# jfkirk/tensorrec

Hardware: NVIDIA H100
Metric: predict_rank_pairs_per_s (higher is better)
Workload: dtype f32 (1 fp16 wgmma filter pass with a certified bound + re-scoring of the survivors from the 22-bit split operands, fp32 accumulate)

## Files before the change

tensorrec_b200/csrc/filter_tc.cuh:

```cuda
#pragma once

#include "common.cuh"

namespace trk {

constexpr uint32_t kWarpStageBytes = 32 * 32 * 4u;
constexpr uint32_t kAccStageBytes = 4 * kWarpStageBytes;
constexpr float kMarginFactor = 1.5f * 0.0009765625f;
constexpr float kBiasUlps = 4.0f * 1.1920929e-7f;
constexpr float kThetaMargins = 2.25f;
constexpr int kGiveUpOverflows = 8;

struct AdmitCtx {
  const float* bias;
  const int32_t* perm;
  int32_t id_offset;
  int32_t n_items;
  int32_t k;
};

template <class Row>
__device__ __forceinline__ void set_tau(Row& r) {
  const float t = (r.theta - r.ubias) * r.inv_c;
  r.tau = t - 8.0f * 1.1920929e-7f * fabsf(t) - 1e-30f;
}

__device__ __forceinline__ float ldg_nc_f32(const float* p) {
  float v;
  asm volatile("ld.global.nc.f32 %0, [%1];" : "=f"(v) : "l"(p));
  return v;
}
__device__ __forceinline__ int32_t ldg_nc_s32(const int32_t* p) {
  int32_t v;
  asm volatile("ld.global.nc.s32 %0, [%1];" : "=r"(v) : "l"(p));
  return v;
}

__device__ __forceinline__ float acc_max_16(const uint32_t* acc, float (&g)[4]) {
#pragma unroll
  for (int q = 0; q < 4; ++q)
    g[q] = fmaxf(fmaxf(__uint_as_float(acc[4 * q]), __uint_as_float(acc[4 * q + 1])),
                 fmaxf(__uint_as_float(acc[4 * q + 2]), __uint_as_float(acc[4 * q + 3])));
  return fmaxf(fmaxf(g[0], g[1]), fmaxf(g[2], g[3]));
}
__device__ __forceinline__ float acc_max_16(const uint32_t* acc) {
  float g[4];
  return acc_max_16(acc, g);
}

__device__ __forceinline__ uint32_t pass_mask_16(const uint32_t* acc, const float (&g)[4], float bmax_scaled,
                                                 float tau) {
  uint32_t mask = 0;
#pragma unroll
  for (int q = 0; q < 4; ++q) {
    if (g[q] + bmax_scaled > tau) {
      const uint32_t b0 = (__uint_as_float(acc[4 * q + 0]) + bmax_scaled > tau) ? (1u << (4 * q + 0)) : 0u;
      const uint32_t b1 = (__uint_as_float(acc[4 * q + 1]) + bmax_scaled > tau) ? (1u << (4 * q + 1)) : 0u;
      const uint32_t b2 = (__uint_as_float(acc[4 * q + 2]) + bmax_scaled > tau) ? (1u << (4 * q + 2)) : 0u;
      const uint32_t b3 = (__uint_as_float(acc[4 * q + 3]) + bmax_scaled > tau) ? (1u << (4 * q + 3)) : 0u;
      mask |= (b0 | b1) | (b2 | b3);
    }
  }
  return mask;
}

__device__ __forceinline__ int filter_owned_row(int warp_in_group, int lane) {
  return 16 * warp_in_group + (lane & 15) + 64 * (lane >> 4);
}

template <int c>
__device__ __forceinline__ float chunk_row_max(const float (&acc0)[32], const float (&acc1)[32], int lane) {
  float m[4];
#pragma unroll
  for (int s = 0; s < 2; ++s) {
    const int i = 16 * c + 2 * s;
    m[s] = fmaxf(fmaxf(fmaxf(acc0[i], acc0[i + 1]), fmaxf(acc0[i + 4], acc0[i + 5])),
                 fmaxf(fmaxf(acc0[i + 8], acc0[i + 9]), fmaxf(acc0[i + 12], acc0[i + 13])));
    m[2 + s] = fmaxf(fmaxf(fmaxf(acc1[i], acc1[i + 1]), fmaxf(acc1[i + 4], acc1[i + 5])),
                     fmaxf(fmaxf(acc1[i + 8], acc1[i + 9]), fmaxf(acc1[i + 12], acc1[i + 13])));
  }
  const bool b0 = (lane & 1) != 0, b1 = (lane & 2) != 0;
  const float k0 = fmaxf(b0 ? m[1] : m[0], __shfl_xor_sync(0xffffffffu, b0 ? m[0] : m[1], 1));
  const float k1 = fmaxf(b0 ? m[3] : m[2], __shfl_xor_sync(0xffffffffu, b0 ? m[2] : m[3], 1));
  const float r = fmaxf(b1 ? k1 : k0, __shfl_xor_sync(0xffffffffu, b1 ? k0 : k1, 2));
  return __shfl_sync(0xffffffffu, r, 4 * (lane & 7) + (lane >> 3));
}

__device__ __forceinline__ uint32_t stage_swizzle(int g) { return 4u * static_cast<uint32_t>(((g & 3) << 1) | (g >> 2)); }
__device__ __forceinline__ void f_sts32(uint32_t addr, float v) {
  asm volatile("st.shared.f32 [%0], %1;" ::"r"(addr), "f"(v) : "memory");
}

template <int c>
__device__ __forceinline__ void stage_warp_chunk(const float (&acc0)[32], const float (&acc1)[32], uint32_t stage,
                                                 int lane) {
  __syncwarp();
  const int g = lane >> 2;
  const uint32_t col0 = 2u * static_cast<uint32_t>(lane & 3) ^ stage_swizzle(g);
  const uint32_t row_g = stage + 128u * g;
#pragma unroll
  for (int j = 0; j < 4; ++j) {
    const uint32_t a = row_g + 4u * (col0 ^ (8u * j));
#pragma unroll
    for (int s = 0; s < 2; ++s) {
      const int i = 16 * c + 4 * j + 2 * s;
      asm volatile("st.shared.v2.f32 [%0], {%1, %2};" ::"r"(a + 1024u * s), "f"(acc0[i]), "f"(acc0[i + 1]) : "memory");
      asm volatile("st.shared.v2.f32 [%0], {%1, %2};" ::"r"(a + 1024u * (2 + s)), "f"(acc1[i]), "f"(acc1[i + 1])
                   : "memory");
    }
  }
  __syncwarp();
}
__device__ __forceinline__ void load_staged_row(uint32_t stage, int lane, uint32_t (&v)[32]) {
  const uint32_t row = stage + 128u * lane, sw = stage_swizzle(lane & 7);
#pragma unroll
  for (uint32_t q = 0; q < 8; ++q)
    asm volatile("ld.shared.v4.b32 {%0, %1, %2, %3}, [%4];"
                 : "=r"(v[4 * q]), "=r"(v[4 * q + 1]), "=r"(v[4 * q + 2]), "=r"(v[4 * q + 3])
                 : "r"(row + 4u * ((4u * q) ^ sw))
                 : "memory");
}

inline __device__ __noinline__ int32_t excl_mask_chunk(const int32_t* indptr, const int32_t* pos, int64_t u,
                                                       int32_t base, uint32_t stage, int lane) {
  const uint32_t row = stage + 128u * lane, sw = stage_swizzle(lane & 7);
  const int hi = __ldg(indptr + u + 1);
  int i = excl_lower_bound(pos, __ldg(indptr + u), hi, base);
  int32_t e = i < hi ? __ldg(pos + i) : 0x7fffffff;
  while (e < base + 32) {
    f_sts32(row + 4u * (static_cast<uint32_t>(e - base) ^ sw), -__int_as_float(0x7f800000));
    ++i;
    e = i < hi ? __ldg(pos + i) : 0x7fffffff;
  }
  return e;
}

template <int kNKB>
__device__ __forceinline__ void filter_mma_half(float (&acc0)[32], float (&acc1)[32], uint32_t a_base, uint32_t b_slot,
                                                int h) {
  wgmma_fence();
#pragma unroll
  for (int kb = 0; kb < kNKB; ++kb) {
#pragma unroll
    for (int ks = 0; ks < kKBlock / kMmaK; ++ks) {
      const uint64_t db = wgmma_desc_k_major_sw128(b_slot + kb * kBTileBytes + h * (kBTileBytes / 2)) + 2u * ks;
      const uint64_t da = wgmma_desc_k_major_sw128(a_base + kb * kATileBytes) + 2u * ks;
      const uint32_t accumulate = static_cast<uint32_t>(kb > 0 || ks > 0);
      wgmma_m64n64k16_f16(acc0, da, db, accumulate);
      wgmma_m64n64k16_f16(acc1, da + ((kATileBytes / 2) >> 4), db, accumulate);
    }
  }
  wgmma_commit();
  wgmma_wait<0>();
}

__device__ __forceinline__ uint32_t wide_key(float s) {
  const uint32_t u = __float_as_uint(s);
  return (u & 0x80000000u) ? ~u : (u | 0x80000000u);
}
__device__ __forceinline__ float wide_unkey(uint32_t key) {
  return __uint_as_float((key & 0x80000000u) ? (key & 0x7fffffffu) : ~key);
}

}
```

tensorrec_b200/csrc/score_filter_tc.cu:

```cuda
#include <stdlib.h>

#include "filter_tc.cuh"

namespace trk {

constexpr int kBufEntries = 32;
constexpr int kKeepMax = 16;
constexpr int kFilterMaxK = 12;

struct FilterParams {
  const __half* user_split;
  const float* user_scale;
  const float* user_bias;
  const float* user_norm;
  const float* item_bias;
  const float* block_bias_max;
  const float* block_bias_min;
  const int32_t* item_perm;
  const float* item_stats;
  int64_t n_users;
  int64_t n_items;
  int32_t n_kblocks;
  int32_t d_pad;
  int32_t n_stages;
  int32_t k;
  int32_t n_splits;
  int32_t tiles_per_split;
  int32_t n_tiles;
  int32_t n_user_pairs;
  int32_t item_id_offset;
  int32_t tile_end_trigger;
  float* cand_score;
  int32_t* cand_item;
  float* row_theta;
  const int32_t* excl_indptr;
  const int32_t* excl_pos;
};

struct FilterLayout {
  uint32_t a_off, b_off, buf_off, acc_off, bar_off, total;
};
__host__ __device__ inline FilterLayout filter_layout(int n_kblocks, int n_stages) {
  FilterLayout L;
  L.a_off = 0;
  L.b_off = L.a_off + 2u * static_cast<uint32_t>(n_kblocks) * kATileBytes;
  L.buf_off = L.b_off + static_cast<uint32_t>(n_stages) * kBTileBytes;
  L.acc_off = L.buf_off + 2u * kBlockM * kBufEntries * 8u;
  L.bar_off = L.acc_off + 2u * kAccStageBytes;
  L.total = L.bar_off + 512u;
  return L;
}

__device__ __forceinline__ void f_sts64(uint32_t addr, float s, int32_t id) {
  asm volatile("st.shared.v2.b32 [%0], {%1, %2};" ::"r"(addr), "r"(__float_as_uint(s)), "r"(id) : "memory");
}
__device__ __forceinline__ void f_lds64(uint32_t addr, float* s, int32_t* id) {
  uint32_t a, b;
  asm volatile("ld.shared.v2.b32 {%0, %1}, [%2];" : "=r"(a), "=r"(b) : "r"(addr) : "memory");
  *s = __uint_as_float(a);
  *id = static_cast<int32_t>(b);
}
__device__ __forceinline__ bool cand_before(float xs, int32_t xi, float ys, int32_t yi) {
  return xs > ys || (xs == ys && xi < yi);
}

struct RowState {
  uint32_t buf;
  int cnt;
  int n_res;
  int n_ovf;
  float tau;
  float theta;
  float drop_max;
  float m3, ubias, c, inv_c;
};


struct RowFetch {
  float s;
  int32_t id;
  float bias;
  int32_t perm;
  int n, n_res;
  uint32_t addr;
};
__device__ __forceinline__ RowFetch compact_fetch(const RowState& r, int lane, int src, const AdmitCtx& ctx) {
  RowFetch f;
  f.n = __shfl_sync(0xffffffffu, r.cnt, src);
  f.n_res = __shfl_sync(0xffffffffu, r.n_res, src);
  f.addr = __shfl_sync(0xffffffffu, r.buf, src);
  f.s = -__int_as_float(0x7f800000);
  f.id = 0x7fffffff;
  f.bias = 0.0f;
  f.perm = 0;
  if (lane < f.n) {
    f_lds64(f.addr + lane * 8, &f.s, &f.id);
    if (lane >= f.n_res) {
      f.bias = ldg_nc_f32(ctx.bias + f.id);
      f.perm = (ctx.perm != nullptr && f.id < ctx.n_items) ? ldg_nc_s32(ctx.perm + f.id) : f.id;
    }
  }
  return f;
}
__device__ __forceinline__ void compact_finish(const RowFetch& f, int lane, int src, RowState& r, const AdmitCtx& ctx) {
  const float kNegInf = -__int_as_float(0x7f800000);
  const int k = ctx.k;
  const int n = f.n;
  const uint32_t addr = f.addr;
  const float m3s = __shfl_sync(0xffffffffu, r.m3, src);
  const float cs = __shfl_sync(0xffffffffu, r.c, src);
  const float ubs = __shfl_sync(0xffffffffu, r.ubias, src);
  float s = f.s;
  int32_t id = f.id;
  if (lane < n && lane >= f.n_res) {
    const int32_t pos = id;
    id = pos < ctx.n_items ? ctx.id_offset + f.perm : 0x7fffffff;
    s = fmaf(s, cs, ubs) + f.bias;
  }
#pragma unroll
  for (int size = 2; size <= 32; size <<= 1) {
#pragma unroll
    for (int stride = size >> 1; stride > 0; stride >>= 1) {
      const float os = __shfl_xor_sync(0xffffffffu, s, stride);
      const int32_t oi = __shfl_xor_sync(0xffffffffu, id, stride);
      const bool lower = (lane & stride) == 0;
      const bool descending = (lane & size) == 0;
      const bool other_first = cand_before(os, oi, s, id);
      const bool take_other = (lower == descending) ? other_first : !other_first;
      if (take_other) {
        s = os;
        id = oi;
      }
    }
  }
  const float kth = __shfl_sync(0xffffffffu, s, k - 1);
  const bool have_k = n >= k;
  const float floor_s = have_k ? kth - m3s : kNegInf;
  const unsigned keep = __ballot_sync(0xffffffffu, lane < n && s >= floor_s);
  int n_keep = __popc(keep);
  const bool ovf = n_keep > kKeepMax;
  n_keep = ovf ? kKeepMax : n_keep;
  const float first_dropped = __shfl_sync(0xffffffffu, s, kKeepMax & 31);
  if (lane < n_keep) f_sts64(addr + lane * 8, s, id);
  if (lane == src) {
    r.cnt = n_keep;
    r.n_res = n_keep;
    if (ovf) {
      r.drop_max = fmaxf(r.drop_max, first_dropped);
      r.n_ovf += 1;
    }
    if (have_k) {
      r.theta = floor_s;
      set_tau(r);
    }
    if (r.n_ovf >= kGiveUpOverflows) {
      r.tau = __int_as_float(0x7f800000);
      r.drop_max = __int_as_float(0x7f800000);
    }
  }
  __syncwarp();
}
__device__ __forceinline__ void compact_rows(unsigned rows, int lane, RowState& r, const AdmitCtx& ctx) {
  if (rows == 0u) return;
  int src = __ffs(rows) - 1;
  rows &= rows - 1;
  RowFetch cur = compact_fetch(r, lane, src, ctx);
  while (true) {
    const int nxt = rows != 0u ? __ffs(rows) - 1 : -1;
    rows &= rows - 1;
    RowFetch ahead = cur;
    if (nxt >= 0) ahead = compact_fetch(r, lane, nxt, ctx);
    compact_finish(cur, lane, src, r, ctx);
    if (nxt < 0) break;
    cur = ahead;
    src = nxt;
  }
}


__device__ __forceinline__ void admit_16(const uint32_t* acc, bool hit, int32_t pos_base, float bmax_scaled, int lane,
                                         RowState& r, const AdmitCtx& ctx) {
  uint32_t pass = 0;
  if (hit) {
#pragma unroll
    for (int j = 0; j < 16; ++j) pass |= (__uint_as_float(acc[j]) + bmax_scaled > r.tau) ? (1u << j) : 0u;
  }
  __syncwarp();
  const unsigned need = __ballot_sync(0xffffffffu, r.cnt + __popc(pass) > kBufEntries);
  compact_rows(need, lane, r, ctx);
  if (pass != 0 && r.n_ovf < kGiveUpOverflows) {
#pragma unroll
    for (int j = 0; j < 16; ++j) {
      if ((pass >> j) & 1u) {
        f_sts64(r.buf + r.cnt * 8, __uint_as_float(acc[j]), pos_base + j);
        r.cnt += 1;
      }
    }
  }
}

__device__ __forceinline__ void append_16(const uint32_t* acc, uint32_t mask, float amax, int32_t pos_base,
                                          RowState& r) {
  if ((mask & (mask - 1u)) == 0u) {
    f_sts64(r.buf + r.cnt * 8, amax, pos_base + __ffs(mask) - 1);
    r.cnt += 1;
  } else {
#pragma unroll
    for (int j = 0; j < 16; ++j) {
      if ((mask >> j) & 1u)
        f_sts64(r.buf + (r.cnt + __popc(mask & ((1u << j) - 1u))) * 8, __uint_as_float(acc[j]), pos_base + j);
    }
    r.cnt += __popc(mask);
  }
}

__device__ __forceinline__ void filter_32(const uint32_t* acc, int32_t pos_base, float bmax_scaled, int lane,
                                          RowState& r, const AdmitCtx& ctx) {
  float g0[4], g1[4];
  const float a0 = acc_max_16(acc, g0), a1 = acc_max_16(acc + 16, g1);
  const bool h0 = a0 + bmax_scaled > r.tau, h1 = a1 + bmax_scaled > r.tau;
  if (__any_sync(0xffffffffu, h0 || h1)) {
    uint32_t lo = 0, hi = 0;
    if (h0) lo = pass_mask_16(acc, g0, bmax_scaled, r.tau);
    if (h1) hi = pass_mask_16(acc + 16, g1, bmax_scaled, r.tau);
    if (__ballot_sync(0xffffffffu, r.cnt + __popc(lo) + __popc(hi) > kBufEntries) == 0u) {
      if (lo != 0u) append_16(acc, lo, a0, pos_base, r);
      if (hi != 0u) append_16(acc + 16, hi, a1, pos_base + 16, r);
    } else {
      admit_16(acc, h0, pos_base, bmax_scaled, lane, r, ctx);
      admit_16(acc + 16, h1, pos_base + 16, bmax_scaled, lane, r, ctx);
    }
  }
}

__device__ __forceinline__ float acc_max_8(const uint32_t* acc) {
  return fmaxf(fmaxf(fmaxf(__uint_as_float(acc[0]), __uint_as_float(acc[1])),
                     fmaxf(__uint_as_float(acc[2]), __uint_as_float(acc[3]))),
               fmaxf(fmaxf(__uint_as_float(acc[4]), __uint_as_float(acc[5])),
                     fmaxf(__uint_as_float(acc[6]), __uint_as_float(acc[7]))));
}
__device__ __forceinline__ void sort16_desc(float (&g)[16]) {
#pragma unroll
  for (int size = 2; size <= 16; size <<= 1) {
#pragma unroll
    for (int stride = size >> 1; stride > 0; stride >>= 1) {
#pragma unroll
      for (int i = 0; i < 16; ++i) {
        const int j = i ^ stride;
        if (j > i) {
          const bool desc = (i & size) == 0;
          const float hi = fmaxf(g[i], g[j]), lo = fminf(g[i], g[j]);
          g[i] = desc ? hi : lo;
          g[j] = desc ? lo : hi;
        }
      }
    }
  }
}


template <int kC, bool kExclude>
__device__ __forceinline__ void filter_chunk(const float (&acc0)[32], const float (&acc1)[32], float amax, int32_t base,
                                             float bmax_scaled, uint32_t stage, int lane, int64_t u,
                                             const FilterParams& p, int32_t& excl_next, RowState& r,
                                             const AdmitCtx& ctx) {
  bool flag = amax + bmax_scaled > r.tau;
  if constexpr (kExclude) flag = flag || excl_next < base + 32;
  if (!__any_sync(0xffffffffu, flag)) return;
  stage_warp_chunk<kC>(acc0, acc1, stage, lane);
  if constexpr (kExclude) {
    if (excl_next < base + 32) excl_next = excl_mask_chunk(p.excl_indptr, p.excl_pos, u, base, stage, lane);
  }
  uint32_t v[32];
  load_staged_row(stage, lane, v);
  filter_32(v, base, bmax_scaled, lane, r, ctx);
}


template <int kNKB, int kCluster, bool kExclude = false>
__global__ void __launch_bounds__(kTcThreads, 1)
score_filter_kernel(const __grid_constant__ CUtensorMap map_users, const __grid_constant__ CUtensorMap map_items,
                    const FilterParams p) {
  uint8_t* smem = smem_base_1024();
  const FilterLayout L = filter_layout(kNKB, p.n_stages);
  const int n_slots = p.n_stages / kNKB;
  uint64_t* bars = reinterpret_cast<uint64_t*>(smem + L.bar_off);
  uint64_t* a_full = bars + 0;
  uint64_t* b_full = bars + 2;
  uint64_t* b_empty = bars + 2 + n_slots;
  constexpr uint32_t kSlotBytes = kNKB * kBTileBytes;

  const int warp = threadIdx.x / 32;
  const int lane = threadIdx.x % 32;
  const uint32_t crank = kCluster == 2 ? cluster_ctarank() : 0u;
  const int n_groups = (p.n_user_pairs + kCluster - 1) / kCluster;
  const int64_t n_work = static_cast<int64_t>(n_groups) * p.n_splits;
  const int64_t w_first = blockIdx.x / kCluster, w_step = gridDim.x / kCluster;
  constexpr uint16_t kClusterMask = (1u << kCluster) - 1u;

  if (warp == 0 && lane == 0) {
    tma_prefetch_desc(&map_items);
    tma_prefetch_desc(&map_users);
  }
  if (warp == 1 && lane == 0) {
    for (int i = 0; i < 2; ++i) mbar_init(a_full + i, 1);
    for (int i = 0; i < n_slots; ++i) {
      mbar_init(b_full + i, 1);
      mbar_init(b_empty + i, 8 * kCluster);
    }
    fence_mbar_init();
  }
  __syncthreads();
  if (kCluster == 2) cluster_sync_all();

  if (warp < 4) {
    asm volatile("setmaxnreg.dec.sync.aligned.u32 40;\n" ::: "memory");
    if (warp == 0) {
      int ts = 0;
      uint32_t ts_phase = 0;
      for (int64_t w = w_first; w < n_work; w += w_step) {
        const int sp = static_cast<int>(w / n_groups);
        const int t0 = sp * p.tiles_per_split;
        const int t1 = min(t0 + p.tiles_per_split, p.n_tiles);
        for (int t = t0; t < t1; ++t) {
          if (kCluster == 2)
            mbar_wait_cluster(b_empty + ts, ts_phase ^ 1);
          else
            mbar_wait(b_empty + ts, ts_phase ^ 1);
          if (elect_one()) {
            mbar_arrive_expect_tx(b_full + ts, kSlotBytes);
#pragma unroll
            for (int kb = 0; kb < kNKB; ++kb) {
              if (kCluster == 2)
                tma_load_2d_multicast(smem + L.b_off + ts * kSlotBytes + kb * kBTileBytes + crank * (kBTileBytes / 2),
                                      &map_items, b_full + ts, kb * kKBlock,
                                      t * kBlockN + static_cast<int>(crank) * (kBlockN / 2), kClusterMask, kEvictLast);
              else
                tma_load_2d(smem + L.b_off + ts * kSlotBytes + kb * kBTileBytes, &map_items, b_full + ts,
                            kb * kKBlock, t * kBlockN, kEvictLast);
            }
          }
          __syncwarp();
          if (++ts == n_slots) {
            ts = 0;
            ts_phase ^= 1;
          }
        }
      }
    }
  } else {
    asm volatile("setmaxnreg.inc.sync.aligned.u32 232;\n" ::: "memory");
    const int group = warp / 4 - 1;
    const int row = filter_owned_row(warp % 4, lane);
    const float kNegInf = -__int_as_float(0x7f800000);
    const uint32_t buf_row_addr =
        smem_u32(smem + L.buf_off) + static_cast<uint32_t>((group * kBlockM + row) * kBufEntries * 8);
    const uint32_t stage = smem_u32(smem + L.acc_off) + static_cast<uint32_t>(warp - 4) * kWarpStageBytes;
    const uint32_t a_base = smem_u32(smem + L.a_off) + group * kNKB * kATileBytes;
    const uint32_t b_base = smem_u32(smem + L.b_off);
    const float max_item_norm = __ldg(p.item_stats + 0);
    const float item_scale = fmaxf(__ldg(p.item_stats + 1), 1e-38f);
    const float max_item_bias = __ldg(p.item_stats + 2);
    const AdmitCtx ctx = {p.item_bias, p.item_perm, p.item_id_offset, static_cast<int32_t>(p.n_items), p.k};
    int ts = 0;
    uint32_t ts_phase = 0, witer = 0;
    float acc0[32], acc1[32];

    for (int64_t w = w_first; w < n_work; w += w_step) {
      const int up = static_cast<int>(w % n_groups) * kCluster + static_cast<int>(crank);
      const int sp = static_cast<int>(w / n_groups);
      const int t0 = sp * p.tiles_per_split;
      const int t1 = min(t0 + p.tiles_per_split, p.n_tiles);
      const int64_t ublock_row0 = (static_cast<int64_t>(up) * 2 + group) * kBlockM;
      const int64_t u = ublock_row0 + row;
      const bool u_ok = u < p.n_users;
      const float su = u_ok ? __ldg(p.user_scale + u) : 1.0f;
      const float ubias = (u_ok && p.user_bias != nullptr) ? __ldg(p.user_bias + u) : 0.0f;
      const float unorm = u_ok ? __ldg(p.user_norm + u) : 0.0f;
      RowState rs;
      rs.buf = buf_row_addr;
      rs.cnt = rs.n_res = rs.n_ovf = 0;
      rs.tau = rs.theta = rs.drop_max = kNegInf;
      rs.ubias = ubias;
      rs.c = su * item_scale;
      rs.inv_c = 1.0f / rs.c;
      rs.m3 = kThetaMargins * (kMarginFactor * unorm * max_item_norm + kBiasUlps * (fabsf(ubias) + max_item_bias));
      int32_t excl_next = 0x7fffffff;
      if constexpr (kExclude) {
        if (u_ok && t1 > t0) excl_next = excl_next_at(p.excl_indptr, p.excl_pos, u, t0 * kBlockN);
      }

      if (t1 > t0) {
        named_barrier_sync(1 + group, kConsumerThreads);
        if (warp % 4 == 0 && lane == 0) {
          mbar_arrive_expect_tx(a_full + group, kNKB * kATileBytes);
#pragma unroll
          for (int kb = 0; kb < kNKB; ++kb)
            tma_load_2d(smem + L.a_off + (group * kNKB + kb) * kATileBytes, &map_users, a_full + group, kb * kKBlock,
                        static_cast<int32_t>(ublock_row0), kEvictFirst);
        }
        mbar_wait(a_full + group, witer & 1);
        ++witer;
      }

      float bmax_next = t1 > t0 ? __ldg(p.block_bias_max + t0) : 0.0f;
      for (int t = t0; t < t1; ++t) {
        const float bmax_scaled = bmax_next * rs.inv_c;
        if (t + 1 < t1) bmax_next = __ldg(p.block_bias_max + t + 1);
        mbar_wait(b_full + ts, ts_phase);
        const uint32_t b_slot = b_base + ts * kSlotBytes;
        const int32_t pos0 = t * kBlockN;
        if (t == t0 && p.block_bias_min != nullptr) {
          const float bmin = __ldg(p.block_bias_min + t0);
          if (bmin > kNegInf) {
            float g[16];
            int32_t pre_next = excl_next;
#pragma unroll
            for (int h = 0; h < 2; ++h) {
              filter_mma_half<kNKB>(acc0, acc1, a_base, b_slot, h);
              uint32_t v[32];
              stage_warp_chunk<0>(acc0, acc1, stage, lane);
              if constexpr (kExclude) {
                if (pre_next < pos0 + h * 64 + 32)
                  pre_next = excl_mask_chunk(p.excl_indptr, p.excl_pos, u, pos0 + h * 64, stage, lane);
              }
              load_staged_row(stage, lane, v);
#pragma unroll
              for (int q = 0; q < 4; ++q) g[8 * h + q] = acc_max_8(v + 8 * q);
              stage_warp_chunk<1>(acc0, acc1, stage, lane);
              if constexpr (kExclude) {
                if (pre_next < pos0 + h * 64 + 64)
                  pre_next = excl_mask_chunk(p.excl_indptr, p.excl_pos, u, pos0 + h * 64 + 32, stage, lane);
              }
              load_staged_row(stage, lane, v);
#pragma unroll
              for (int q = 0; q < 4; ++q) g[8 * h + 4 + q] = acc_max_8(v + 8 * q);
            }
            sort16_desc(g);
            float a_k = g[0];
#pragma unroll
            for (int i = 1; i < 16; ++i) a_k = (i < p.k) ? g[i] : a_k;
            const float th0 = (fmaf(a_k, rs.c, ubias) + bmin) - rs.m3;
            if (th0 == th0) {
              rs.theta = th0;
              set_tau(rs);
            }
          }
        }
#pragma unroll 1
        for (int h = 0; h < 2; ++h) {
          filter_mma_half<kNKB>(acc0, acc1, a_base, b_slot, h);
          if (h == 1) {
            __syncwarp();
            if (lane == 0) {
              if (kCluster == 2) {
#pragma unroll
                for (uint32_t r = 0; r < kCluster; ++r) mbar_arrive_cluster(b_empty + ts, r);
              } else {
                mbar_arrive(b_empty + ts);
              }
            }
          }
          const float amax0 = chunk_row_max<0>(acc0, acc1, lane), amax1 = chunk_row_max<1>(acc0, acc1, lane);
          filter_chunk<0, kExclude>(acc0, acc1, amax0, pos0 + h * 64, bmax_scaled, stage, lane, u, p, excl_next, rs,
                                    ctx);
          filter_chunk<1, kExclude>(acc0, acc1, amax1, pos0 + h * 64 + 32, bmax_scaled, stage, lane, u, p, excl_next,
                                    rs, ctx);
        }
        if (++ts == n_slots) {
          ts = 0;
          ts_phase ^= 1;
        }
        {
          const unsigned early = __ballot_sync(0xffffffffu, rs.cnt > p.tile_end_trigger);
          compact_rows(early, lane, rs, ctx);
        }
      }

      compact_rows(0xffffffffu, lane, rs, ctx);
      if (u_ok) {
        const int64_t base = u * p.n_splits + sp;
        float* os = p.cand_score + base * kKeepMax;
        int32_t* oi = p.cand_item + base * kKeepMax;
        for (int e = 0; e < kKeepMax; ++e) {
          float s = kNegInf;
          int32_t id = 0x7fffffff;
          if (e < rs.cnt) f_lds64(rs.buf + e * 8, &s, &id);
          os[e] = s;
          oi[e] = id;
        }
        const bool th_nan = rs.theta != rs.theta || rs.drop_max != rs.drop_max;
        p.row_theta[base] = th_nan ? __int_as_float(0x7f800000) : fmaxf(rs.theta, rs.drop_max);
      }
      __syncwarp();
    }
  }

  __syncthreads();
  if (kCluster == 2) cluster_sync_all();
}

__global__ void operand_stats_kernel(const __half* __restrict__ split, const float* __restrict__ scale, int64_t rows,
                                     int d_pad, float* __restrict__ out_norm, float* __restrict__ stats) {
  const int lane = threadIdx.x % 32;
  const int64_t warp = (static_cast<int64_t>(blockIdx.x) * blockDim.x + threadIdx.x) / 32;
  const int64_t n_warps = static_cast<int64_t>(gridDim.x) * blockDim.x / 32;
  float local_max_norm = 0.0f, local_max_scale = 0.0f;
  for (int64_t r = warp; r < rows; r += n_warps) {
    const __half* hi = split + r * 2 * d_pad;
    const __half* lo = hi + d_pad;
    float ss = 0.0f;
    for (int e = lane * 2; e < d_pad; e += 64) {
      const float2 h = __half22float2(*reinterpret_cast<const __half2*>(hi + e));
      const float2 l = __half22float2(*reinterpret_cast<const __half2*>(lo + e));
      const float x0 = h.x + l.x, x1 = h.y + l.y;
      ss = fmaf(x0, x0, ss);
      ss = fmaf(x1, x1, ss);
    }
#pragma unroll
    for (int o = 16; o > 0; o >>= 1) ss += __shfl_xor_sync(0xffffffffu, ss, o);
    const float sc = scale[r];
    const float norm = sqrtf(ss) * sc * 1.002f;
    if (lane == 0) {
      if (out_norm != nullptr) out_norm[r] = norm;
      local_max_norm = fmaxf(local_max_norm, norm);
      if (ss > 0.0f) local_max_scale = fmaxf(local_max_scale, sc);
    }
  }
  if (lane == 0 && stats != nullptr) {
    atomicMax(reinterpret_cast<int*>(stats + 0), __float_as_int(local_max_norm));
    atomicMax(reinterpret_cast<int*>(stats + 1), __float_as_int(local_max_scale));
  }
}

__global__ void rescale_hi_global_kernel(const __half* __restrict__ split, const float* __restrict__ scale,
                                         const float* __restrict__ stats, const int32_t* __restrict__ perm,
                                         int64_t rows, int d_pad, __half* __restrict__ out_hi) {
  const float inv_max = 1.0f / fmaxf(stats[1], 1e-38f);
  const int64_t n_vec = rows * (d_pad / 8);
  for (int64_t i = static_cast<int64_t>(blockIdx.x) * blockDim.x + threadIdx.x; i < n_vec;
       i += static_cast<int64_t>(gridDim.x) * blockDim.x) {
    const int64_t r = i / (d_pad / 8);
    const int e = static_cast<int>(i % (d_pad / 8)) * 8;
    const int64_t src = perm != nullptr ? perm[r] : r;
    const float f = scale[src] * inv_max;
    uint4 raw = *reinterpret_cast<const uint4*>(split + src * 2 * d_pad + e);
    __half2* h = reinterpret_cast<__half2*>(&raw);
#pragma unroll
    for (int q = 0; q < 4; ++q) {
      const float2 v = __half22float2(h[q]);
      h[q] = __floats2half2_rn(v.x * f, v.y * f);
    }
    *reinterpret_cast<uint4*>(out_hi + r * d_pad + e) = raw;
  }
}

__global__ void invert_perm_kernel(const int32_t* __restrict__ perm, int64_t n, int32_t* __restrict__ inv) {
  for (int64_t i = static_cast<int64_t>(blockIdx.x) * blockDim.x + threadIdx.x; i < n;
       i += static_cast<int64_t>(gridDim.x) * blockDim.x)
    inv[perm[i]] = static_cast<int32_t>(i);
}
__global__ void exclusion_keys_kernel(const int32_t* __restrict__ indptr, const int32_t* __restrict__ ids,
                                      const int32_t* __restrict__ inv, int64_t rows, int64_t* __restrict__ keys) {
  const int lane = threadIdx.x % 32;
  const int64_t warp = (static_cast<int64_t>(blockIdx.x) * blockDim.x + threadIdx.x) / 32;
  const int64_t n_warps = static_cast<int64_t>(gridDim.x) * blockDim.x / 32;
  for (int64_t r = warp; r < rows; r += n_warps) {
    const int e1 = indptr[r + 1];
    for (int e = indptr[r] + lane; e < e1; e += 32) {
      const int32_t pos = inv != nullptr ? inv[ids[e]] : ids[e];
      keys[e] = static_cast<int64_t>(static_cast<uint64_t>(r) << 32 | static_cast<uint32_t>(pos));
    }
  }
}

int score_filter_max_k() { return kFilterMaxK; }
int score_filter_list_width() { return kKeepMax; }

int operand_stats(const void* split, const float* scale, int64_t rows, int32_t d_pad, float* out_norm, float* stats,
                  cudaStream_t stream) {
  TRK_CHECK_ARG(split && scale && rows >= 0 && d_pad >= 64 && d_pad % 64 == 0, "operand_stats: bad arguments");
  if (rows == 0) return TRK_OK;
  const int threads = 256;
  operand_stats_kernel<<<capped_grid(ceil_div(rows, threads / 32), 8), threads, 0, stream>>>(
      static_cast<const __half*>(split), scale, rows, d_pad, out_norm, stats);
  TRK_CHECK_LAUNCH();
  return TRK_OK;
}

int rescale_hi_global(const void* split, const float* scale, const float* stats, const int32_t* perm, int64_t rows,
                      int32_t d_pad, void* out_hi, cudaStream_t stream) {
  TRK_CHECK_ARG(split && scale && stats && out_hi && rows >= 0 && d_pad >= 64 && d_pad % 64 == 0,
                "rescale_hi_global: bad arguments");
  if (rows == 0) return TRK_OK;
  const int threads = 256;
  rescale_hi_global_kernel<<<capped_grid(ceil_div(rows * (d_pad / 8), threads), 16), threads, 0, stream>>>(
      static_cast<const __half*>(split), scale, stats, perm, rows, d_pad, static_cast<__half*>(out_hi));
  TRK_CHECK_LAUNCH();
  return TRK_OK;
}

int exclusion_positions(const int32_t* item_perm, int64_t n_items, int32_t* inv_perm, const int32_t* excl_indptr,
                        const int32_t* excl_ids, int64_t n_rows, int64_t* out_keys, cudaStream_t stream) {
  TRK_CHECK_ARG(excl_indptr && excl_ids && out_keys && n_rows >= 0 && n_items >= 0, "exclusion_positions: bad arguments");
  TRK_CHECK_ARG(item_perm == nullptr || inv_perm != nullptr, "exclusion_positions: item_perm needs inv_perm");
  if (item_perm != nullptr && n_items > 0) {
    invert_perm_kernel<<<capped_grid(ceil_div(n_items, 256), 16), 256, 0, stream>>>(item_perm, n_items, inv_perm);
    TRK_CHECK_LAUNCH();
  }
  if (n_rows == 0) return TRK_OK;
  exclusion_keys_kernel<<<capped_grid(ceil_div(n_rows, 256 / 32), 16), 256, 0, stream>>>(
      excl_indptr, excl_ids, item_perm != nullptr ? inv_perm : nullptr, n_rows, out_keys);
  TRK_CHECK_LAUNCH();
  return TRK_OK;
}

int score_filter_f16(const void* user_split, const float* user_scale, const float* user_bias,
                     const float* user_norm, const void* item_hi, const float* item_stats, const float* item_bias,
                     const float* block_bias_max, const float* block_bias_min, const int32_t* item_perm,
                     int64_t n_users, int64_t n_items, int32_t d_pad, int32_t k, int32_t n_splits,
                     int32_t item_id_offset, float* cand_score, int32_t* cand_item, float* row_theta,
                     const int32_t* excl_indptr, const int32_t* excl_pos, cudaStream_t stream) {
  TRK_CHECK_ARG(user_split && user_scale && user_norm && item_hi && item_stats && item_bias && block_bias_max,
                "score_filter: null input");
  TRK_CHECK_ARG((excl_indptr == nullptr) == (excl_pos == nullptr), "score_filter: excl_indptr and excl_pos go together");
  TRK_CHECK_ARG(cand_score && cand_item && row_theta, "score_filter: null output");
  TRK_CHECK_ARG(n_users >= 1 && n_items >= 1 && n_splits >= 1, "score_filter: empty shape");
  TRK_CHECK_ARG(n_users < (1ll << 31) && n_items < (1ll << 31) - 512, "score_filter: shape exceeds int32 indexing");
  if (d_pad != 64 && d_pad != 128) {
    set_error("score_filter: d_pad=%d not supported (64 or 128)", d_pad);
    return TRK_ERR_UNSUPPORTED;
  }
  if (k < 1 || k > kFilterMaxK) {
    set_error("score_filter: k=%d outside [1, %d]", k, kFilterMaxK);
    return TRK_ERR_UNSUPPORTED;
  }
  TRK_CHECK_ARG(reinterpret_cast<uintptr_t>(user_split) % 16 == 0 && reinterpret_cast<uintptr_t>(item_hi) % 16 == 0 &&
                    reinterpret_cast<uintptr_t>(item_bias) % 16 == 0,
                "score_filter: operands must be 16-byte aligned");

  FilterParams p;
  p.user_split = static_cast<const __half*>(user_split);
  p.d_pad = d_pad;
  p.user_scale = user_scale;
  p.user_bias = user_bias;
  p.user_norm = user_norm;
  p.item_bias = item_bias;
  p.block_bias_max = block_bias_max;
  p.block_bias_min = block_bias_min;
  p.item_perm = item_perm;
  p.item_stats = item_stats;
  p.n_users = n_users;
  p.n_items = n_items;
  p.n_kblocks = d_pad / kKBlock;
  p.k = k;
  p.n_tiles = static_cast<int32_t>(ceil_div(n_items, kBlockN));
  p.n_splits = n_splits;
  p.tiles_per_split = static_cast<int32_t>(ceil_div(p.n_tiles, n_splits));
  p.n_user_pairs = static_cast<int32_t>(ceil_div(n_users, 2 * kBlockM));
  p.item_id_offset = item_id_offset;
  p.tile_end_trigger = 26;
  {
    const char* env = getenv("TRK_FILTER_TILE_END_TRIGGER");
    if (env != nullptr) p.tile_end_trigger = atoi(env) < kBufEntries ? atoi(env) : kBufEntries;
    if (p.tile_end_trigger < kKeepMax + 2) p.tile_end_trigger = kKeepMax + 2;
  }
  p.cand_score = cand_score;
  p.cand_item = cand_item;
  p.row_theta = row_theta;
  p.excl_indptr = excl_indptr;
  p.excl_pos = excl_pos;
  const bool excl = excl_indptr != nullptr;
  CUtensorMap map_users, map_items;
  int rc;
  p.n_stages = 0;
  for (int s = kMaxStages; s >= 2; --s)
    if (s % p.n_kblocks == 0 && filter_layout(p.n_kblocks, s).total + kSmemAlignSlack <= kSmemLimit) {
      p.n_stages = s;
      break;
    }
  TRK_CHECK_ARG(p.n_stages >= 2 * p.n_kblocks, "score_filter: shared memory budget exceeded");
  const uint32_t smem_bytes = filter_layout(p.n_kblocks, p.n_stages).total + kSmemAlignSlack;

  int cluster = 2;
  {
    const char* env = getenv("TRK_FILTER_CLUSTER");
    if (env != nullptr && (atoi(env) == 1 || atoi(env) == 2)) cluster = atoi(env);
  }
  auto kernel2 = excl ? (p.n_kblocks == 2 ? score_filter_kernel<2, 2, true> : score_filter_kernel<1, 2, true>)
                     : (p.n_kblocks == 2 ? score_filter_kernel<2, 2> : score_filter_kernel<1, 2>);
  auto kernel1 = excl ? (p.n_kblocks == 2 ? score_filter_kernel<2, 1, true> : score_filter_kernel<1, 1, true>)
                     : (p.n_kblocks == 2 ? score_filter_kernel<2, 1> : score_filter_kernel<1, 1>);
  cudaLaunchConfig_t cfg = {};
  cudaLaunchAttribute attr[1];
  int max_clusters = 0;
  if (cluster == 2) {
    TRK_CHECK_CUDA(cudaFuncSetAttribute(kernel2, cudaFuncAttributeMaxDynamicSharedMemorySize, smem_bytes));
    cfg.gridDim = dim3(2);
    cfg.blockDim = dim3(kTcThreads);
    cfg.dynamicSmemBytes = smem_bytes;
    cfg.stream = stream;
    attr[0].id = cudaLaunchAttributeClusterDimension;
    attr[0].val.clusterDim.x = 2;
    attr[0].val.clusterDim.y = 1;
    attr[0].val.clusterDim.z = 1;
    cfg.attrs = attr;
    cfg.numAttrs = 1;
    static int cached_clusters[64][4];
    static bool cached_valid[64][4];
    int device = 0;
    TRK_CHECK_CUDA(cudaGetDevice(&device));
    const int variant = (p.n_kblocks == 2 ? 1 : 0) + (excl ? 2 : 0);
    if (device >= 0 && device < 64 && cached_valid[device][variant]) {
      max_clusters = cached_clusters[device][variant];
    } else {
      if (cudaOccupancyMaxActiveClusters(&max_clusters, kernel2, &cfg) != cudaSuccess) {
        (void)cudaGetLastError();
        max_clusters = 0;
      }
      if (device >= 0 && device < 64) {
        cached_clusters[device][variant] = max_clusters;
        cached_valid[device][variant] = true;
      }
    }
    const char* env = getenv("TRK_FILTER_CLUSTER");
    if (max_clusters * 2 < sm_count() - 8 && env == nullptr) cluster = 1;
    if (max_clusters < 1) cluster = 1;
  }
  rc = encode_tiled_2d(&map_items, CU_TENSOR_MAP_DATA_TYPE_FLOAT16, item_hi, d_pad, n_items, 2 * d_pad, kKBlock,
                       kBlockN / cluster, CU_TENSOR_MAP_L2_PROMOTION_L2_256B);
  if (rc != TRK_OK) return rc;
  rc = encode_tiled_2d(&map_users, CU_TENSOR_MAP_DATA_TYPE_FLOAT16, user_split, d_pad, n_users, 4 * d_pad, kKBlock,
                       kBlockM, CU_TENSOR_MAP_L2_PROMOTION_L2_256B);
  if (rc != TRK_OK) return rc;
  if (cluster == 2) {
    const int64_t n_work = ceil_div(static_cast<int64_t>(p.n_user_pairs), 2) * n_splits;
    const int n_clusters = static_cast<int>(n_work < max_clusters ? n_work : max_clusters);
    cfg.gridDim = dim3(static_cast<unsigned>(2 * n_clusters));
    TRK_CHECK_CUDA(cudaLaunchKernelEx(&cfg, kernel2, map_users, map_items, p));
  } else {
    TRK_CHECK_CUDA(cudaFuncSetAttribute(kernel1, cudaFuncAttributeMaxDynamicSharedMemorySize, smem_bytes));
    const int grid = capped_grid(static_cast<int64_t>(p.n_user_pairs) * n_splits, 1);
    kernel1<<<grid, kTcThreads, smem_bytes, stream>>>(map_users, map_items, p);
  }
  TRK_CHECK_LAUNCH();
  return TRK_OK;
}

}
```

Measured before the change: 2063 billion.

## Split filter wgmma by row halves using m64n128 tiles and per-fragment threshold checks

The filter pass used to issue two m64n64 wgmmas per column half, one for each 64-row half of the A tile. It now issues one m64n128 wgmma per 64-row half covering all item columns, so each B tile is read once per row half with a wider N. The chunk pass test now compares fragment maxima against per-row thresholds gathered by shuffles instead of doing a full cross-lane row max. Staging and ownership masks change so that only half the lanes own rows in each pass. The per-row staging and filter work is now done twice, once per row half, which risks more serialized shared-memory and shuffle work and fewer active lanes in each pass.

```diff
diff --git a/tensorrec_b200/csrc/filter_tc.cuh b/tensorrec_b200/csrc/filter_tc.cuh
--- a/tensorrec_b200/csrc/filter_tc.cuh
+++ b/tensorrec_b200/csrc/filter_tc.cuh
@@ -68,22 +68,22 @@
   return 16 * warp_in_group + (lane & 15) + 64 * (lane >> 4);
 }
 
-template <int c>
-__device__ __forceinline__ float chunk_row_max(const float (&acc0)[32], const float (&acc1)[32], int lane) {
-  float m[4];
+__device__ __forceinline__ void frag_rows(float x, int rh, int lane, float (&f)[2]) {
+  f[0] = __shfl_sync(0xffffffffu, x, 16 * rh + (lane >> 2));
+  f[1] = __shfl_sync(0xffffffffu, x, 16 * rh + 8 + (lane >> 2));
+}
+
+template <int c>
+__device__ __forceinline__ bool chunk_frag_pass(const float (&acc)[64], const float (&bf)[2], const float (&tf)[2]) {
+  bool pass = false;
 #pragma unroll
   for (int s = 0; s < 2; ++s) {
     const int i = 16 * c + 2 * s;
-    m[s] = fmaxf(fmaxf(fmaxf(acc0[i], acc0[i + 1]), fmaxf(acc0[i + 4], acc0[i + 5])),
-                 fmaxf(fmaxf(acc0[i + 8], acc0[i + 9]), fmaxf(acc0[i + 12], acc0[i + 13])));
-    m[2 + s] = fmaxf(fmaxf(fmaxf(acc1[i], acc1[i + 1]), fmaxf(acc1[i + 4], acc1[i + 5])),
-                     fmaxf(fmaxf(acc1[i + 8], acc1[i + 9]), fmaxf(acc1[i + 12], acc1[i + 13])));
-  }
-  const bool b0 = (lane & 1) != 0, b1 = (lane & 2) != 0;
-  const float k0 = fmaxf(b0 ? m[1] : m[0], __shfl_xor_sync(0xffffffffu, b0 ? m[0] : m[1], 1));
-  const float k1 = fmaxf(b0 ? m[3] : m[2], __shfl_xor_sync(0xffffffffu, b0 ? m[2] : m[3], 1));
-  const float r = fmaxf(b1 ? k1 : k0, __shfl_xor_sync(0xffffffffu, b1 ? k0 : k1, 2));
-  return __shfl_sync(0xffffffffu, r, 4 * (lane & 7) + (lane >> 3));
+    const float m = fmaxf(fmaxf(fmaxf(acc[i], acc[i + 1]), fmaxf(acc[i + 4], acc[i + 5])),
+                          fmaxf(fmaxf(acc[i + 8], acc[i + 9]), fmaxf(acc[i + 12], acc[i + 13])));
+    pass = pass || m + bf[s] > tf[s];
+  }
+  return pass;
 }
 
 __device__ __forceinline__ uint32_t stage_swizzle(int g) { return 4u * static_cast<uint32_t>(((g & 3) << 1) | (g >> 2)); }
@@ -92,21 +92,18 @@
 }
 
 template <int c>
-__device__ __forceinline__ void stage_warp_chunk(const float (&acc0)[32], const float (&acc1)[32], uint32_t stage,
-                                                 int lane) {
+__device__ __forceinline__ void stage_warp_chunk(const float (&acc)[64], int rh, uint32_t stage, int lane) {
   __syncwarp();
   const int g = lane >> 2;
   const uint32_t col0 = 2u * static_cast<uint32_t>(lane & 3) ^ stage_swizzle(g);
-  const uint32_t row_g = stage + 128u * g;
+  const uint32_t row_g = stage + 2048u * static_cast<uint32_t>(rh) + 128u * g;
 #pragma unroll
   for (int j = 0; j < 4; ++j) {
     const uint32_t a = row_g + 4u * (col0 ^ (8u * j));
 #pragma unroll
     for (int s = 0; s < 2; ++s) {
       const int i = 16 * c + 4 * j + 2 * s;
-      asm volatile("st.shared.v2.f32 [%0], {%1, %2};" ::"r"(a + 1024u * s), "f"(acc0[i]), "f"(acc0[i + 1]) : "memory");
-      asm volatile("st.shared.v2.f32 [%0], {%1, %2};" ::"r"(a + 1024u * (2 + s)), "f"(acc1[i]), "f"(acc1[i + 1])
-                   : "memory");
+      asm volatile("st.shared.v2.f32 [%0], {%1, %2};" ::"r"(a + 1024u * s), "f"(acc[i]), "f"(acc[i + 1]) : "memory");
     }
   }
   __syncwarp();
@@ -136,6 +133,63 @@
 }
 
 template <int kNKB>
+__device__ __forceinline__ void filter_mma_rows(float (&acc)[64], uint32_t a_base, uint32_t b_slot, int rh) {
+  wgmma_fence();
+#pragma unroll
+  for (int kb = 0; kb < kNKB; ++kb) {
+#pragma unroll
+    for (int ks = 0; ks < kKBlock / kMmaK; ++ks) {
+      const uint64_t db = wgmma_desc_k_major_sw128(b_slot + kb * kBTileBytes) + 2u * ks;
+      const uint64_t da = wgmma_desc_k_major_sw128(a_base + kb * kATileBytes) + 2u * ks +
+                          static_cast<uint32_t>(rh) * ((kATileBytes / 2) >> 4);
+      wgmma_m64n128k16_f16(acc, da, db, static_cast<uint32_t>(kb > 0 || ks > 0));
+    }
+  }
+  wgmma_commit();
+  wgmma_wait<0>();
+}
+
+
+template <int c>
+__device__ __forceinline__ float chunk_row_max(const float (&acc0)[32], const float (&acc1)[32], int lane) {
+  float m[4];
+#pragma unroll
+  for (int s = 0; s < 2; ++s) {
+    const int i = 16 * c + 2 * s;
+    m[s] = fmaxf(fmaxf(fmaxf(acc0[i], acc0[i + 1]), fmaxf(acc0[i + 4], acc0[i + 5])),
+                 fmaxf(fmaxf(acc0[i + 8], acc0[i + 9]), fmaxf(acc0[i + 12], acc0[i + 13])));
+    m[2 + s] = fmaxf(fmaxf(fmaxf(acc1[i], acc1[i + 1]), fmaxf(acc1[i + 4], acc1[i + 5])),
+                     fmaxf(fmaxf(acc1[i + 8], acc1[i + 9]), fmaxf(acc1[i + 12], acc1[i + 13])));
+  }
+  const bool b0 = (lane & 1) != 0, b1 = (lane & 2) != 0;
+  const float k0 = fmaxf(b0 ? m[1] : m[0], __shfl_xor_sync(0xffffffffu, b0 ? m[0] : m[1], 1));
+  const float k1 = fmaxf(b0 ? m[3] : m[2], __shfl_xor_sync(0xffffffffu, b0 ? m[2] : m[3], 1));
+  const float r = fmaxf(b1 ? k1 : k0, __shfl_xor_sync(0xffffffffu, b1 ? k0 : k1, 2));
+  return __shfl_sync(0xffffffffu, r, 4 * (lane & 7) + (lane >> 3));
+}
+
+template <int c>
+__device__ __forceinline__ void stage_warp_chunk(const float (&acc0)[32], const float (&acc1)[32], uint32_t stage,
+                                                 int lane) {
+  __syncwarp();
+  const int g = lane >> 2;
+  const uint32_t col0 = 2u * static_cast<uint32_t>(lane & 3) ^ stage_swizzle(g);
+  const uint32_t row_g = stage + 128u * g;
+#pragma unroll
+  for (int j = 0; j < 4; ++j) {
+    const uint32_t a = row_g + 4u * (col0 ^ (8u * j));
+#pragma unroll
+    for (int s = 0; s < 2; ++s) {
+      const int i = 16 * c + 4 * j + 2 * s;
+      asm volatile("st.shared.v2.f32 [%0], {%1, %2};" ::"r"(a + 1024u * s), "f"(acc0[i]), "f"(acc0[i + 1]) : "memory");
+      asm volatile("st.shared.v2.f32 [%0], {%1, %2};" ::"r"(a + 1024u * (2 + s)), "f"(acc1[i]), "f"(acc1[i + 1])
+                   : "memory");
+    }
+  }
+  __syncwarp();
+}
+
+template <int kNKB>
 __device__ __forceinline__ void filter_mma_half(float (&acc0)[32], float (&acc1)[32], uint32_t a_base, uint32_t b_slot,
                                                 int h) {
   wgmma_fence();
diff --git a/tensorrec_b200/csrc/score_filter_tc.cu b/tensorrec_b200/csrc/score_filter_tc.cu
--- a/tensorrec_b200/csrc/score_filter_tc.cu
+++ b/tensorrec_b200/csrc/score_filter_tc.cu
@@ -214,11 +214,11 @@
   }
 }
 
-__device__ __forceinline__ void filter_32(const uint32_t* acc, int32_t pos_base, float bmax_scaled, int lane,
+__device__ __forceinline__ void filter_32(const uint32_t* acc, bool own, int32_t pos_base, float bmax_scaled, int lane,
                                           RowState& r, const AdmitCtx& ctx) {
   float g0[4], g1[4];
   const float a0 = acc_max_16(acc, g0), a1 = acc_max_16(acc + 16, g1);
-  const bool h0 = a0 + bmax_scaled > r.tau, h1 = a1 + bmax_scaled > r.tau;
+  const bool h0 = own && a0 + bmax_scaled > r.tau, h1 = own && a1 + bmax_scaled > r.tau;
   if (__any_sync(0xffffffffu, h0 || h1)) {
     uint32_t lo = 0, hi = 0;
     if (h0) lo = pass_mask_16(acc, g0, bmax_scaled, r.tau);
@@ -260,20 +260,51 @@
 
 
 template <int kC, bool kExclude>
-__device__ __forceinline__ void filter_chunk(const float (&acc0)[32], const float (&acc1)[32], float amax, int32_t base,
-                                             float bmax_scaled, uint32_t stage, int lane, int64_t u,
+__device__ __forceinline__ void filter_chunk(const float (&acc)[64], int rh, int32_t base, float bmax_scaled,
+                                             const float (&bf)[2], float (&tf)[2], uint32_t stage, int lane, int64_t u,
                                              const FilterParams& p, int32_t& excl_next, RowState& r,
                                              const AdmitCtx& ctx) {
-  bool flag = amax + bmax_scaled > r.tau;
-  if constexpr (kExclude) flag = flag || excl_next < base + 32;
+  const bool own = (lane >> 4) == rh;
+  bool flag = chunk_frag_pass<kC>(acc, bf, tf);
+  if constexpr (kExclude) flag = flag || (own && excl_next < base + 32);
   if (!__any_sync(0xffffffffu, flag)) return;
-  stage_warp_chunk<kC>(acc0, acc1, stage, lane);
+  stage_warp_chunk<kC>(acc, rh, stage, lane);
   if constexpr (kExclude) {
-    if (excl_next < base + 32) excl_next = excl_mask_chunk(p.excl_indptr, p.excl_pos, u, base, stage, lane);
+    if (own && excl_next < base + 32) excl_next = excl_mask_chunk(p.excl_indptr, p.excl_pos, u, base, stage, lane);
   }
   uint32_t v[32];
   load_staged_row(stage, lane, v);
-  filter_32(v, base, bmax_scaled, lane, r, ctx);
+  filter_32(v, own, base, bmax_scaled, lane, r, ctx);
+  frag_rows(r.tau, rh, lane, tf);
+}
+
+template <bool kExclude>
+__device__ __forceinline__ void filter_row_half(const float (&acc)[64], int rh, int32_t pos0, float bmax_scaled,
+                                                uint32_t stage, int lane, int64_t u, const FilterParams& p,
+                                                int32_t& excl_next, RowState& r, const AdmitCtx& ctx) {
+  float bf[2], tf[2];
+  frag_rows(bmax_scaled, rh, lane, bf);
+  frag_rows(r.tau, rh, lane, tf);
+  filter_chunk<0, kExclude>(acc, rh, pos0, bmax_scaled, bf, tf, stage, lane, u, p, excl_next, r, ctx);
+  filter_chunk<1, kExclude>(acc, rh, pos0 + 32, bmax_scaled, bf, tf, stage, lane, u, p, excl_next, r, ctx);
+  filter_chunk<2, kExclude>(acc, rh, pos0 + 64, bmax_scaled, bf, tf, stage, lane, u, p, excl_next, r, ctx);
+  filter_chunk<3, kExclude>(acc, rh, pos0 + 96, bmax_scaled, bf, tf, stage, lane, u, p, excl_next, r, ctx);
+}
+
+template <int kC, bool kExclude>
+__device__ __forceinline__ void warm_chunk(const float (&acc)[64], int rh, int32_t pos0, uint32_t stage, int lane,
+                                           int64_t u, const FilterParams& p, int32_t& pre_next, float (&g)[16]) {
+  const bool own = (lane >> 4) == rh;
+  stage_warp_chunk<kC>(acc, rh, stage, lane);
+  if constexpr (kExclude) {
+    if (own && pre_next < pos0 + 32 * kC + 32)
+      pre_next = excl_mask_chunk(p.excl_indptr, p.excl_pos, u, pos0 + 32 * kC, stage, lane);
+  }
+  uint32_t v[32];
+  load_staged_row(stage, lane, v);
+#pragma unroll
+  for (int q = 0; q < 4; ++q)
+    if (own) g[4 * kC + q] = acc_max_8(v + 8 * q);
 }
 
 
@@ -364,7 +395,7 @@
     const AdmitCtx ctx = {p.item_bias, p.item_perm, p.item_id_offset, static_cast<int32_t>(p.n_items), p.k};
     int ts = 0;
     uint32_t ts_phase = 0, witer = 0;
-    float acc0[32], acc1[32];
+    float acc[64];
 
     for (int64_t w = w_first; w < n_work; w += w_step) {
       const int up = static_cast<int>(w % n_groups) * kCluster + static_cast<int>(crank);
@@ -416,25 +447,12 @@
             float g[16];
             int32_t pre_next = excl_next;
 #pragma unroll
-            for (int h = 0; h < 2; ++h) {
-              filter_mma_half<kNKB>(acc0, acc1, a_base, b_slot, h);
-              uint32_t v[32];
-              stage_warp_chunk<0>(acc0, acc1, stage, lane);
-              if constexpr (kExclude) {
-                if (pre_next < pos0 + h * 64 + 32)
-                  pre_next = excl_mask_chunk(p.excl_indptr, p.excl_pos, u, pos0 + h * 64, stage, lane);
-              }
-              load_staged_row(stage, lane, v);
-#pragma unroll
-              for (int q = 0; q < 4; ++q) g[8 * h + q] = acc_max_8(v + 8 * q);
-              stage_warp_chunk<1>(acc0, acc1, stage, lane);
-              if constexpr (kExclude) {
-                if (pre_next < pos0 + h * 64 + 64)
-                  pre_next = excl_mask_chunk(p.excl_indptr, p.excl_pos, u, pos0 + h * 64 + 32, stage, lane);
-              }
-              load_staged_row(stage, lane, v);
-#pragma unroll
-              for (int q = 0; q < 4; ++q) g[8 * h + 4 + q] = acc_max_8(v + 8 * q);
+            for (int rh = 0; rh < 2; ++rh) {
+              filter_mma_rows<kNKB>(acc, a_base, b_slot, rh);
+              warm_chunk<0, kExclude>(acc, rh, pos0, stage, lane, u, p, pre_next, g);
+              warm_chunk<1, kExclude>(acc, rh, pos0, stage, lane, u, p, pre_next, g);
+              warm_chunk<2, kExclude>(acc, rh, pos0, stage, lane, u, p, pre_next, g);
+              warm_chunk<3, kExclude>(acc, rh, pos0, stage, lane, u, p, pre_next, g);
             }
             sort16_desc(g);
             float a_k = g[0];
@@ -448,9 +466,9 @@
           }
         }
 #pragma unroll 1
-        for (int h = 0; h < 2; ++h) {
-          filter_mma_half<kNKB>(acc0, acc1, a_base, b_slot, h);
-          if (h == 1) {
+        for (int rh = 0; rh < 2; ++rh) {
+          filter_mma_rows<kNKB>(acc, a_base, b_slot, rh);
+          if (rh == 1) {
             __syncwarp();
             if (lane == 0) {
               if (kCluster == 2) {
@@ -461,11 +479,12 @@
               }
             }
           }
-          const float amax0 = chunk_row_max<0>(acc0, acc1, lane), amax1 = chunk_row_max<1>(acc0, acc1, lane);
-          filter_chunk<0, kExclude>(acc0, acc1, amax0, pos0 + h * 64, bmax_scaled, stage, lane, u, p, excl_next, rs,
-                                    ctx);
-          filter_chunk<1, kExclude>(acc0, acc1, amax1, pos0 + h * 64 + 32, bmax_scaled, stage, lane, u, p, excl_next,
-                                    rs, ctx);
+          bool excl_rh = false;
+          if constexpr (kExclude) excl_rh = __any_sync(0xffffffffu, (lane >> 4) == rh && excl_next < pos0 + kBlockN);
+          if (excl_rh)
+            filter_row_half<kExclude>(acc, rh, pos0, bmax_scaled, stage, lane, u, p, excl_next, rs, ctx);
+          else
+            filter_row_half<false>(acc, rh, pos0, bmax_scaled, stage, lane, u, p, excl_next, rs, ctx);
         }
         if (++ts == n_slots) {
           ts = 0;
```

After: 2134 billion (median of 6 runs). 1.03x the previous value.
